# Hanbo-Cheng/DAWN-pytorch

Hardware: AMD Instinct MI355X
Metric: generated frames/sec at 256x256, 50 DDIM steps (higher is better)
Workload: dtype f32

## Files before the change

dawn-pytorch_amd/csrc/cond_xattn.hip:

```cpp
#include "dawn_common.h"
#include "../../include/dawn_hip.h"

namespace {

constexpr int XH = 8, XD = 8;
constexpr float XSCALE = 8.0f;

__global__ void xattn_prep_kernel(const float* __restrict__ kv, int F, const float* __restrict__ k_scale,
                                  const float* __restrict__ null_kv, float* __restrict__ kvtab, int branch,
                                  float* __restrict__ nulltab) {
    const int t = blockIdx.x * blockDim.x + threadIdx.x;
    if (t < F * XH) {
        const int f = t / XH, h = t % XH;
        const float* k = kv + (long)f * 128 + h * XD;
        const float* v = kv + (long)f * 128 + 64 + h * XD;
        float n2 = 0.f;
#pragma unroll
        for (int d = 0; d < XD; ++d) n2 += k[d] * k[d];
        const float inv = 1.0f / fmaxf(sqrtf(n2), 1e-12f);
        float* o = kvtab + ((long)f * 3 + branch) * 128;
#pragma unroll
        for (int d = 0; d < XD; ++d) {
            o[h * XD + d] = k[d] * inv * k_scale[d];
            o[64 + h * XD + d] = v[d];
// ... 57 lines not shown
__global__ __launch_bounds__(256) void xattn_ln_sum_kernel(const float* __restrict__ y3, const float* __restrict__ g3,
                                                           float* __restrict__ out, long rows, int Co, float eps) {
    constexpr int RPB = 256 / L;
    constexpr int MAXQ = 2;
    const int sub = threadIdx.x % L;
    const long row = (long)blockIdx.x * RPB + threadIdx.x / L;
    const bool ok = row < rows;
    const int nq = Co >> 2;
    f32x4 acc[MAXQ];
#pragma unroll
    for (int i = 0; i < MAXQ; ++i) acc[i] = f32x4{0.f, 0.f, 0.f, 0.f};
    for (int b = 0; b < 3; ++b) {
        const float* y = y3 + (row * 3 + b) * Co;
        f32x4 v[MAXQ];
        float s = 0.f;
#pragma unroll
        for (int i = 0; i < MAXQ; ++i) {
            const int qd = sub + i * L;
            v[i] = f32x4{0.f, 0.f, 0.f, 0.f};
            if (ok && qd < nq) {
                v[i] = *reinterpret_cast<const f32x4*>(y + qd * 4);
                s += v[i].x + v[i].y + v[i].z + v[i].w;
            }
        }
        s = wave_sum(s, L);
        const float mu = s / (float)Co;
        float ss = 0.f;
#pragma unroll
        for (int i = 0; i < MAXQ; ++i) {
            const int qd = sub + i * L;
            if (ok && qd < nq) {
                const f32x4 dl = v[i] - mu;
                ss += dl.x * dl.x + dl.y * dl.y + dl.z * dl.z + dl.w * dl.w;
            }
        }
        ss = wave_sum(ss, L);
        const float rs = rsqrtf(ss / (float)Co + eps);
#pragma unroll
        for (int i = 0; i < MAXQ; ++i) {
            const int qd = sub + i * L;
            if (ok && qd < nq) {
                const f32x4 g = *reinterpret_cast<const f32x4*>(g3 + b * Co + qd * 4);
                acc[i] += (v[i] - mu) * rs * g;
            }
        }
    }
#pragma unroll
    for (int i = 0; i < MAXQ; ++i) {
        const int qd = sub + i * L;
        if (ok && qd < nq) *reinterpret_cast<f32x4*>(out + row * Co + qd * 4) = acc[i];
    }
}

template <int L, int MAXQ>
__global__ __launch_bounds__(256) void xattn_sigma_out_kernel(const float* __restrict__ q, long rows, int HW,
                                                              const float* __restrict__ xtab, const float* __restrict__ g3,
                                                              int Co, float eps, float* out,
                                                              const float* gn_x , const float* __restrict__ gn_a,
                                                              const float* __restrict__ gn_b) {
    constexpr int RPB = 256 / L, R = 4;
    const int sub = threadIdx.x % L;
    const int lane = threadIdx.x & 63;
    const int gbase = lane - sub;
    const long row0 = ((long)blockIdx.x * RPB + threadIdx.x / L) * R;
    if (row0 >= rows) return;
    const int nq = Co >> 2;
    const int W = 64 + 9 * Co;
    const float* xt = xtab + (row0 / HW) * 3 * W;
    const int hd = sub & 7;
    f32x4 acc[R][MAXQ];
#pragma unroll
    for (int r = 0; r < R; ++r)
#pragma unroll
        for (int i = 0; i < MAXQ; ++i) acc[r][i] = f32x4{0.f, 0.f, 0.f, 0.f};
    const float rCo = 1.0f / (float)Co;
#pragma unroll 1
    for (int b = 0; b < 3; ++b) {
        const float* tb = xt + b * W;
        const f32x4 d0 = *reinterpret_cast<const f32x4*>(tb + hd * 8), d1 = *reinterpret_cast<const f32x4*>(tb + hd * 8 + 4);
        f32x4 u[9][MAXQ], g[MAXQ];
#pragma unroll
        for (int i = 0; i < MAXQ; ++i) {
            const int qd = sub + i * L;
            const bool ok = qd < nq;
#pragma unroll
            for (int k = 0; k < 9; ++k)
                u[k][i] = ok ? *reinterpret_cast<const f32x4*>(tb + 64 + k * Co + qd * 4) : f32x4{0.f, 0.f, 0.f, 0.f};
            g[i] = ok ? *reinterpret_cast<const f32x4*>(g3 + b * Co + qd * 4) : f32x4{0.f, 0.f, 0.f, 0.f};
        }
#pragma unroll
        for (int r = 0; r < R; ++r) {
            const float* qr = q + (row0 + r) * 192 + b * 64 + hd * 8;
            const f32x4 q0 = *reinterpret_cast<const f32x4*>(qr), q1 = *reinterpret_cast<const f32x4*>(qr + 4);
            const float n2 = (q0.x * q0.x + q0.y * q0.y + q0.z * q0.z + q0.w * q0.w) + (q1.x * q1.x + q1.y * q1.y + q1.z * q1.z + q1.w * q1.w);
            const float dd = (q0.x * d0.x + q0.y * d0.y + q0.z * d0.z + q0.w * d0.w) + (q1.x * d1.x + q1.y * d1.y + q1.z * d1.z + q1.w * d1.w);
            const float sg = __builtin_amdgcn_rcpf(1.0f + __builtin_amdgcn_exp2f(dd * __builtin_amdgcn_rsqf(fmaxf(n2, 1e-24f))));
            f32x4 y[MAXQ];
#pragma unroll
            for (int i = 0; i < MAXQ; ++i) y[i] = u[8][i];
#pragma unroll
            for (int k = 0; k < 8; ++k) {
                const float sk = __shfl(sg, gbase + k, 64);
#pragma unroll
                for (int i = 0; i < MAXQ; ++i) y[i] += u[k][i] * sk;
            }
            float s1 = 0.f;
#pragma unroll
            for (int i = 0; i < MAXQ; ++i) s1 += (y[i].x + y[i].y) + (y[i].z + y[i].w);
            const float mu = wave_sum(s1, L) * rCo;
            float s2 = 0.f;
#pragma unroll
            for (int i = 0; i < MAXQ; ++i) {
                if (sub + i * L < nq) {
                    const f32x4 dl = y[i] - mu;
                    s2 += (dl.x * dl.x + dl.y * dl.y) + (dl.z * dl.z + dl.w * dl.w);
                }
            }
            const float rs = __builtin_amdgcn_rsqf(wave_sum(s2, L) * rCo + eps);
#pragma unroll
            for (int i = 0; i < MAXQ; ++i) acc[r][i] += (y[i] - mu) * rs * g[i];
        }
    }
#pragma unroll
    for (int r = 0; r < R; ++r)
#pragma unroll
        for (int i = 0; i < MAXQ; ++i) {
            const int qd = sub + i * L;
            if (qd < nq) {
                f32x4 v = acc[r][i];
                if (gn_x) {
                    const f32x4 c4 = *reinterpret_cast<const f32x4*>(gn_x + (row0 + r) * Co + qd * 4);
                    const f32x4 a4 = *reinterpret_cast<const f32x4*>(gn_a + qd * 4), b4 = *reinterpret_cast<const f32x4*>(gn_b + qd * 4);
#pragma unroll
                    for (int j = 0; j < 4; ++j) v[j] = dawn_silu(c4[j] * a4[j] + b4[j]) + v[j];
                }
                *reinterpret_cast<f32x4*>(out + (row0 + r) * Co + qd * 4) = v;
            }
        }
}

}

extern "C" int dawn_xattn_sigma_out_h1(const float* q, long rows, int HW, const float* xtab, const float* g3, int Co, float eps,
                                       const float* gn_x, const float* gn_a, const float* gn_b, float* out, void* stream) {
    if (gn_x && (!gn_a || !gn_b)) return dawn_set_error_msg(-54, "dawn_xattn_sigma_out_h1: gn_x needs gn_a and gn_b");
    if (Co % 32 != 0 || Co < 32 || Co > 512 || HW % 4 != 0 || rows % 4 != 0)
        return dawn_set_error_msg(-53, "dawn_xattn_sigma_out: need Co % 32 == 0, 32 <= Co <= 512, H*W % 4 == 0");
    if (rows <= 0) return 0;
    hipStream_t s = (hipStream_t)stream;
    const int nq = Co / 4;
#define LAUNCH_XS(L, MQ)                                                                                                   \
    hipLaunchKernelGGL((xattn_sigma_out_kernel<L, MQ>), dim3(dawn_cdiv(rows, (256 / L) * 4)), dim3(256), 0, s, q, rows, HW, xtab, \
                       g3, Co, eps, out, gn_x, gn_a, gn_b)
    if (nq > 64) LAUNCH_XS(64, 2);
    else if (nq > 32) LAUNCH_XS(64, 1);
    else if (nq > 16) LAUNCH_XS(32, 1);
    else if (nq > 8) LAUNCH_XS(16, 1);
    else LAUNCH_XS(8, 1);
#undef LAUNCH_XS
    DAWN_LAUNCH_CHECK();
    return 0;
}
extern "C" int dawn_xattn_sigma_out(const float* q, long rows, int HW, const float* xtab, const float* g3, int Co, float eps,
                                    float* out, void* stream) {
    return dawn_xattn_sigma_out_h1(q, rows, HW, xtab, g3, Co, eps, nullptr, nullptr, nullptr, out, stream);
}

extern "C" int dawn_xattn_prep(const float* kv, int F, const float* k_scale, const float* null_kv, float* kvtab,
                               int branch, float* nulltab, void* stream) {
    hipLaunchKernelGGL(xattn_prep_kernel, dim3(dawn_cdiv((long)F * XH, 256)), dim3(256), 0, (hipStream_t)stream, kv, F,
                       k_scale, null_kv, kvtab, branch, nulltab);
    DAWN_LAUNCH_CHECK();
    return 0;
}
extern "C" int dawn_xattn_core(const float* q, float* o, long rows, int HW, const float* kvtab, const float* nulltab,
                               const float* q_scale, void* stream) {
    long total = rows * 24;
    int grid = (int)((total + 255) / 256);
    if (grid > 16384) grid = 16384;
    hipLaunchKernelGGL(xattn_core_kernel, dim3(grid), dim3(256), 0, (hipStream_t)stream, q, o, rows, HW, kvtab,
                       nulltab, q_scale);
    DAWN_LAUNCH_CHECK();
    return 0;
}
extern "C" int dawn_xattn_ln_sum(const float* y3, const float* g3, float* out, long rows, int Co, float eps,
                                 void* stream) {
    if (Co > 512 || Co % 4 != 0 || Co < 16) return dawn_set_error_msg(-50, "dawn_xattn_ln_sum: need 16 <= Co <= 512");
    hipStream_t s = (hipStream_t)stream;
    const int nq = Co / 4;
#define LAUNCH_XL(L)                                                                                            \
    hipLaunchKernelGGL(xattn_ln_sum_kernel<L>, dim3(dawn_cdiv(rows, 256 / L)), dim3(256), 0, s, y3, g3, out, rows, \
                       Co, eps)
    if (nq >= 64) LAUNCH_XL(64);
    else if (nq >= 32) LAUNCH_XL(32);
    else if (nq >= 16) LAUNCH_XL(16);
    else if (nq >= 8) LAUNCH_XL(8);
    else LAUNCH_XL(4);
#undef LAUNCH_XL
    DAWN_LAUNCH_CHECK();
    return 0;
}
```

dawn-pytorch_amd/csrc/sla_layer.hip:

```cpp
#include "dawn_common.h"
#include "../../include/dawn_hip.h"

namespace {

constexpr int C = 64;
constexpr int HEADS = 8;
constexpr int DH = 32;
constexpr int XLD = 68;
constexpr int QKVN = 3 * HEADS * DH;

__device__ __forceinline__ void stage_tile(const float* __restrict__ xf, int n0, int HW, float eps, float* Xt, int tid) {
    const int px = tid >> 4, sub = tid & 15;
    const int n = n0 + px;
    f32x4 v = {0.f, 0.f, 0.f, 0.f};
    if (n < HW) v = *reinterpret_cast<const f32x4*>(xf + (long)n * C + sub * 4);
    float s = v.x + v.y + v.z + v.w;
    s = wave_sum(s, 16);
    const float mu = s * (1.0f / C);
    const f32x4 dl = v - mu;
    float ss = dl.x * dl.x + dl.y * dl.y + dl.z * dl.z + dl.w * dl.w;
    ss = wave_sum(ss, 16);
    const float rs = 1.0f / sqrtf(ss * (1.0f / C) + eps);
    f32x4 o = dl * rs;
    if (n >= HW) o = f32x4{0.f, 0.f, 0.f, 0.f};
// ... 52 lines not shown
    stage_tile(xf, 0, HW, eps, Xs[0], tid);
    __syncthreads();
    for (int t = 0; t < ntiles; ++t) {
        if (t + 1 < ntiles) stage_tile(xf, 32 * (t + 1), HW, eps, Xs[(t + 1) & 1], tid);
        f32x16 kt = proj_N(Xs[t & 1], l31, half, wk);
        const f32x16 vt = proj_N(Xs[t & 1], l31, half, wv);
#pragma unroll
        for (int r = 0; r < 16; ++r) {
            const int n = 32 * t + (r & 3) + 8 * (r >> 2) + 4 * half;
            const float e = n < HW ? expf(kt[r] - mx) : 0.f;
            kt[r] = e;
            den += e;
        }
#pragma unroll
        for (int r = 0; r < 16; ++r) ctx = __builtin_amdgcn_mfma_f32_32x32x2f32(kt[r], vt[r], ctx, 0, 0, 0);
        __syncthreads();
    }
    den += __shfl_xor(den, 32, 64);
    float* dens = Xs[0];
    if (half == 0) dens[h * 32 + l31] = 1.0f / den;
    __syncthreads();
    float* ct = cT[h];
#pragma unroll
    for (int r = 0; r < 16; ++r) {
        const int d = (r & 3) + 8 * (r >> 2) + 4 * half;
        ct[d * 36 + l31] = ctx[r] * dens[h * 32 + d];
    }
    __syncthreads();
#pragma unroll
    for (int nt = 0; nt < 2; ++nt) {
        f32x16 m = zero16();
#pragma unroll
        for (int c = 0; c < 4; ++c) {
            const f32x4 a4 = *reinterpret_cast<const f32x4*>(ct + l31 * 36 + 8 * c + 4 * half);
            const f32x4 b4 = *reinterpret_cast<const f32x4*>(wout + ((size_t)(h * 8 + 2 * c + half) * C + 32 * nt + l31) * 4);
#pragma unroll
            for (int s = 0; s < 4; ++s) m = __builtin_amdgcn_mfma_f32_32x32x2f32(a4[s], b4[s], m, 0, 0, 0);
        }
        float* mo = Mout + (long)f * (HEADS * 8 * C * 4);
#pragma unroll
        for (int g = 0; g < 4; ++g)
            *reinterpret_cast<f32x4*>(mo + ((size_t)(h * 8 + 2 * g + half) * C + 32 * nt + l31) * 4) =
                f32x4{m[4 * g], m[4 * g + 1], m[4 * g + 2], m[4 * g + 3]};
    }
}


__device__ __forceinline__ f32x4 stage_load(const float* __restrict__ xf, int n0, int HW, int tid) {
    const int n = n0 + (tid >> 4);
    f32x4 v = {0.f, 0.f, 0.f, 0.f};
    if (n < HW) v = *reinterpret_cast<const f32x4*>(xf + (long)n * C + (tid & 15) * 4);
    return v;
}
__device__ __forceinline__ void stage_store(const f32x4 v, int n0, int HW, float eps, unsigned char* Pt, int tid) {
    const int px = tid >> 4, sub = tid & 15;
    const int n = n0 + px;
    float s = v.x + v.y + v.z + v.w;
    s = wave_sum(s, 16);
    const float mu = s * (1.0f / C);
    const f32x4 dl = v - mu;
    float ss = dl.x * dl.x + dl.y * dl.y + dl.z * dl.z + dl.w * dl.w;
    ss = wave_sum(ss, 16);
    const float rs = 1.0f / sqrtf(ss * (1.0f / C) + eps);
    f32x4 o = dl * rs;
    if (n >= HW) o = f32x4{0.f, 0.f, 0.f, 0.f};
    uint2 p1, p2, p3;
    dawn_split3_rne_quad(o, p1, p2, p3);
    const int kc = sub >> 2, qd = sub & 3;
    unsigned char* dst = Pt + ((size_t)((kc * 2 + (qd >> 1)) * 32 + px)) * 16 + (qd & 1) * 8;
    *reinterpret_cast<uint2*>(dst) = p1;
    *reinterpret_cast<uint2*>(dst + 4096) = p2;
    *reinterpret_cast<uint2*>(dst + 8192) = p3;
}

__global__ __launch_bounds__(512) void sla_c64_apply_kernel(const float* x , int HW,
                                                            const float* __restrict__ wqkv,
                                                            const float* __restrict__ Mg, const float* __restrict__ bias,
                                                            float eps, float* out, int nsplit) {
    extern __shared__ __attribute__((aligned(16))) float smem[];
    float* Wq = smem;
    float* Ms = smem + 16 * 256 * 4;
    const int tid = threadIdx.x;
    const int wave = tid >> 6, lane = tid & 63;
    const int l31 = lane & 31, half = lane >> 5;
    const int f = blockIdx.x / nsplit, sp = blockIdx.x % nsplit;
    for (int i = tid; i < 16 * 256; i += 512) {
        const int kq = i >> 8, n = i & 255;
        *reinterpret_cast<f32x4*>(Wq + i * 4) = *reinterpret_cast<const f32x4*>(wqkv + ((size_t)kq * QKVN + n) * 4);
    }
    const float* mf = Mg + (long)f * (HEADS * 8 * C * 4);
    for (int i = tid; i < 64 * 64; i += 512)
        *reinterpret_cast<f32x4*>(Ms + i * 4) = *reinterpret_cast<const f32x4*>(mf + (size_t)i * 4);
    __syncthreads();

    const int ntiles = (HW + 31) >> 5;
    const int per = (ntiles + nsplit - 1) / nsplit;
    const int t0 = sp * per, t1 = min(ntiles, t0 + per);
    const float scale = 0.17677669529663687f;
    for (int t = t0 + wave; t < t1; t += 8) {
        const int n = 32 * t + l31;
        const int nc = n < HW ? n : HW - 1;
        const float* xr = x + ((long)f * HW + nc) * C + 4 * half;
        f32x4 xb[8];
        float s = 0.f;
#pragma unroll
        for (int c = 0; c < 8; ++c) {
            xb[c] = *reinterpret_cast<const f32x4*>(xr + 8 * c);
            s += xb[c].x + xb[c].y + xb[c].z + xb[c].w;
        }
        s += __shfl_xor(s, 32, 64);
        const float mu = s * (1.0f / C);
        float ss = 0.f;
#pragma unroll
        for (int c = 0; c < 8; ++c) {
            const f32x4 dl = xb[c] - mu;
            ss += dl.x * dl.x + dl.y * dl.y + dl.z * dl.z + dl.w * dl.w;
        }
        ss += __shfl_xor(ss, 32, 64);
        const float rs = 1.0f / sqrtf(ss * (1.0f / C) + eps);
        f32x4 xn[8];
#pragma unroll
        for (int c = 0; c < 8; ++c) xn[c] = (xb[c] - mu) * rs;

        f32x16 oT[2];
        oT[0] = zero16();
// ... 178 lines not shown
                }
                l += __shfl_xor(l, 32, 64);
                const float inv = scale * __builtin_amdgcn_rcpf(l);
                if constexpr (OUTB) {
#pragma unroll
                    for (int j = 0; j < 2; ++j) {
                        float q8[8];
#pragma unroll
                        for (int i = 0; i < 8; ++i) q8[i] = qT[8 * j + i] * inv;
                        bf16x8 qb[3];
                        dawn_split3_oct(q8, qb[0], qb[1], qb[2]);
#pragma unroll
                        for (int nt = 0; nt < 2; ++nt) {
                            bf16x8 ma[3];
#pragma unroll
                            for (int pl = 0; pl < 3; ++pl)
                                ma[pl] = *reinterpret_cast<const bf16x8*>(Mp + ((size_t)((((h * 2 + j) * 3 + pl) * 2 + half) * C + 32 * nt + l31)) * 16);
#pragma unroll
                            for (int u = 0; u < 6; ++u)
                                oT[nt] = __builtin_amdgcn_mfma_f32_32x32x16_bf16(ma[DAWN_SPLIT6_A[u]], qb[DAWN_SPLIT6_B[u]], oT[nt], 0, 0, 0);
                        }
                    }
                } else {
#pragma unroll
                    for (int nt = 0; nt < 2; ++nt)
#pragma unroll
                        for (int c = 0; c < 4; ++c) {
                            const f32x4 a4 = *reinterpret_cast<const f32x4*>(Ms + ((h * 8 + 2 * c + half) * C + 32 * nt + l31) * 4);
#pragma unroll
                            for (int s2 = 0; s2 < 4; ++s2)
                                oT[nt] = __builtin_amdgcn_mfma_f32_32x32x2f32(a4[s2], qT[4 * c + s2] * inv, oT[nt], 0, 0, 0);
                        }
                }
            }
            if (n < HW) {
                const float* xrow = x + ((long)f * HW + n) * C;
                float* orow = out + ((long)f * HW + n) * C;
#pragma unroll
                for (int nt = 0; nt < 2; ++nt)
#pragma unroll
                    for (int g2 = 0; g2 < 4; ++g2) {
                        const int ch = 32 * nt + 8 * g2 + 4 * half;
                        const f32x4 b4 = *reinterpret_cast<const f32x4*>(bias + ch);
                        const f32x4 xres = *reinterpret_cast<const f32x4*>(xrow + ch);
                        f32x4 o = {oT[nt][4 * g2], oT[nt][4 * g2 + 1], oT[nt][4 * g2 + 2], oT[nt][4 * g2 + 3]};
                        *reinterpret_cast<f32x4*>(orow + ch) = o + b4 + xres;
                    }
            }
        }
        g += tB - tA;
    }
}

constexpr int SLA_PART = HEADS * (DH * DH + 2 * DH);

__device__ __forceinline__ void sla_ctx_proj(const unsigned char* Pt, int l31, int half, const bf16x8 (&wk)[4][3],
                                             const bf16x8 (&wv)[4][3], f32x16& kt, f32x16& vt) {
    kt = zero16();
    vt = zero16();
#pragma unroll
    for (int kc = 0; kc < 4; ++kc) {
        bf16x8 xa[3];
#pragma unroll
        for (int pl = 0; pl < 3; ++pl)
            xa[pl] = *reinterpret_cast<const bf16x8*>(Pt + pl * 4096 + ((size_t)((kc * 2 + half) * 32 + l31)) * 16);
#pragma unroll
        for (int u = 0; u < 6; ++u) {
            kt = __builtin_amdgcn_mfma_f32_32x32x16_bf16(xa[DAWN_SPLIT6_A[u]], wk[kc][DAWN_SPLIT6_B[u]], kt, 0, 0, 0);
            vt = __builtin_amdgcn_mfma_f32_32x32x16_bf16(xa[DAWN_SPLIT6_A[u]], wv[kc][DAWN_SPLIT6_B[u]], vt, 0, 0, 0);
        }
    }
}

template <bool FULL>
__device__ __forceinline__ void sla_ctx_post(f32x16& kt, const f32x16& vt, int t, int HW, int half, f32x16& ctx, float& den,
                                             float& mx) {
    constexpr float LOG2E = 1.4426950408889634f;
    float tm = -3.0e38f;
#pragma unroll
    for (int r = 0; r < 16; ++r) {
        const int n = 32 * t + (r & 3) + 8 * (r >> 2) + 4 * half;
        if (FULL || n < HW) tm = fmaxf(tm, kt[r]);
    }
    tm = fmaxf(tm, __shfl_xor(tm, 32, 64)) * LOG2E;
    if (__builtin_amdgcn_ballot_w64(tm > mx + 8.0f) != 0ull) {
        const float mnew = fmaxf(mx, tm);
        const float alpha = __builtin_amdgcn_exp2f(mx - mnew);
        den *= alpha;
#pragma unroll
        for (int r = 0; r < 16; ++r) {
            const int d0 = (r & 3) + 8 * (r >> 2);
            const float a0 = __builtin_bit_cast(float, __builtin_amdgcn_readlane(__builtin_bit_cast(int, alpha), d0));
            const float a1 = __builtin_bit_cast(float, __builtin_amdgcn_readlane(__builtin_bit_cast(int, alpha), d0 + 4));
            ctx[r] *= half ? a1 : a0;
        }
        mx = mnew;
    }
#pragma unroll
    for (int r = 0; r < 16; ++r) {
        const int n = 32 * t + (r & 3) + 8 * (r >> 2) + 4 * half;
        float e = __builtin_amdgcn_exp2f(__builtin_fmaf(kt[r], LOG2E, -mx));
        if (!FULL) e = n < HW ? e : 0.f;
        kt[r] = e;
        den += e;
    }
#pragma unroll
    for (int j = 0; j < 2; ++j) {
        float ek[8], vv[8];
#pragma unroll
        for (int i = 0; i < 8; ++i) { ek[i] = kt[8 * j + i]; vv[i] = vt[8 * j + i]; }
        bf16x8 e3[3], v3[3];
        dawn_split3_oct(ek, e3[0], e3[1], e3[2]);
        dawn_split3_oct(vv, v3[0], v3[1], v3[2]);
#pragma unroll
        for (int u = 0; u < 6; ++u) ctx = __builtin_amdgcn_mfma_f32_32x32x16_bf16(e3[DAWN_SPLIT6_A[u]], v3[DAWN_SPLIT6_B[u]], ctx, 0, 0, 0);
    }
}

__global__ __launch_bounds__(512) void sla_c64_context_part_kernel(const float* __restrict__ x, int HW,
                                                                   const unsigned short* __restrict__ wqkv_s, float eps,
                                                                   float* __restrict__ part, int ns, int per) {
    __shared__ __attribute__((aligned(16))) unsigned char Ps[2][12288];
    const int tid = threadIdx.x;
    const int h = tid >> 6, lane = tid & 63;
    const int l31 = lane & 31, half = lane >> 5;
    const int f = blockIdx.x / ns, sl = blockIdx.x - f * ns;
    const float* xf = x + (long)f * HW * C;
    const int ntiles = (HW + 31) >> 5;
    const int tA = sl * per, tB = min(ntiles, tA + per);

    bf16x8 wk[4][3], wv[4][3];
#pragma unroll
    for (int kc = 0; kc < 4; ++kc)
#pragma unroll
        for (int pl = 0; pl < 3; ++pl) {
            const size_t base = ((size_t)((kc * 3 + pl) * 2 + half) * QKVN) * 8;
            wk[kc][pl] = *reinterpret_cast<const bf16x8*>(wqkv_s + base + (size_t)(HEADS * DH + h * DH + l31) * 8);
            wv[kc][pl] = *reinterpret_cast<const bf16x8*>(wqkv_s + base + (size_t)(2 * HEADS * DH + h * DH + l31) * 8);
        }

    f32x16 ctx = zero16();
    float den = 0.f, mx = -3.0e38f;
    f32x4 vnext = {0.f, 0.f, 0.f, 0.f};
    if (tA < tB) stage_store(stage_load(xf, 32 * tA, HW, tid), 32 * tA, HW, eps, Ps[0], tid);
    if (tA + 1 < tB) vnext = stage_load(xf, 32 * (tA + 1), HW, tid);
    __syncthreads();
    f32x16 kt, vt;
    auto post = [&](int t) {
        if (32 * t + 32 <= HW) sla_ctx_post<true>(kt, vt, t, HW, half, ctx, den, mx);
        else sla_ctx_post<false>(kt, vt, t, HW, half, ctx, den, mx);
    };
    if (h < 4) {
        for (int t = tA; t < tB; ++t) {
            const f32x4 vcur = vnext;
            if (t + 2 < tB) vnext = stage_load(xf, 32 * (t + 2), HW, tid);
            sla_ctx_proj(Ps[(t - tA) & 1], l31, half, wk, wv, kt, vt);
            post(t);
            if (t + 1 < tB) stage_store(vcur, 32 * (t + 1), HW, eps, Ps[(t + 1 - tA) & 1], tid);
            __syncthreads();
        }
    } else {
        for (int t = tA; t < tB; ++t) {
            const f32x4 vcur = vnext;
            if (t + 2 < tB) vnext = stage_load(xf, 32 * (t + 2), HW, tid);
            if (t > tA) post(t - 1);
            if (t + 1 < tB) stage_store(vcur, 32 * (t + 1), HW, eps, Ps[(t + 1 - tA) & 1], tid);
            sla_ctx_proj(Ps[(t - tA) & 1], l31, half, wk, wv, kt, vt);
            __syncthreads();
        }
        if (tA < tB) post(tB - 1);
    }
    den += __shfl_xor(den, 32, 64);
    float* P = part + ((long)f * ns + sl) * SLA_PART;
#pragma unroll
    for (int r = 0; r < 16; ++r) {
        const int d = (r & 3) + 8 * (r >> 2) + 4 * half;
        P[h * (DH * DH) + d * DH + l31] = ctx[r];
    }
    if (half == 0) {
        P[HEADS * DH * DH + h * DH + l31] = den;
        P[HEADS * DH * DH + HEADS * DH + h * DH + l31] = mx;
    }
}

__global__ __launch_bounds__(512) void sla_c64_context_merge_kernel(const float* __restrict__ part, int ns,
                                                                    const float* __restrict__ wout, float* __restrict__ Mout) {
    __shared__ __attribute__((aligned(16))) float cT[HEADS][32 * 36];
    const int tid = threadIdx.x;
    const int h = tid >> 6, lane = tid & 63;
    const int l31 = lane & 31, half = lane >> 5;
    const int f = blockIdx.x;
    const float* P0 = part + (long)f * ns * SLA_PART;
    float* ct = cT[h];
    constexpr int OD = HEADS * DH * DH, OM = OD + HEADS * DH;
    float m[16], den[16], acc[16];
#pragma unroll
    for (int i = 0; i < 16; ++i) { m[i] = -3.0e38f; den[i] = 0.f; acc[i] = 0.f; }
    for (int sl = 0; sl < ns; ++sl) {
        const float* P = P0 + (long)sl * SLA_PART;
#pragma unroll
        for (int i = 0; i < 16; ++i) m[i] = fmaxf(m[i], P[OM + h * DH + 2 * i + half]);
    }
    for (int sl = 0; sl < ns; ++sl) {
        const float* P = P0 + (long)sl * SLA_PART;
#pragma unroll
        for (int i = 0; i < 16; ++i) {
            const int d = 2 * i + half;
            const float a = __builtin_amdgcn_exp2f(P[OM + h * DH + d] - m[i]);
            den[i] += a * P[OD + h * DH + d];
            acc[i] += a * P[h * (DH * DH) + d * DH + l31];
        }
    }
#pragma unroll
    for (int i = 0; i < 16; ++i) ct[(2 * i + half) * 36 + l31] = acc[i] * (1.0f / den[i]);
    __syncthreads();
#pragma unroll
    for (int nt = 0; nt < 2; ++nt) {
        f32x16 m = zero16();
#pragma unroll
        for (int c = 0; c < 4; ++c) {
            const f32x4 a4 = *reinterpret_cast<const f32x4*>(ct + l31 * 36 + 8 * c + 4 * half);
            const f32x4 b4 = *reinterpret_cast<const f32x4*>(wout + ((size_t)(h * 8 + 2 * c + half) * C + 32 * nt + l31) * 4);
#pragma unroll
            for (int s = 0; s < 4; ++s) m = __builtin_amdgcn_mfma_f32_32x32x2f32(a4[s], b4[s], m, 0, 0, 0);
        }
        float* mo = Mout + (long)f * (HEADS * 8 * C * 4);
#pragma unroll
        for (int g = 0; g < 4; ++g)
            *reinterpret_cast<f32x4*>(mo + ((size_t)(h * 8 + 2 * g + half) * C + 32 * nt + l31) * 4) =
                f32x4{m[4 * g], m[4 * g + 1], m[4 * g + 2], m[4 * g + 3]};
    }
}

int sla_ncu() {
    static int ncu = 0;
    if (!ncu) {
        int dev = 0, n = 0;
        if (hipGetDevice(&dev) != hipSuccess || hipDeviceGetAttribute(&n, hipDeviceAttributeMultiprocessorCount, dev) != hipSuccess || n <= 0)
            n = 256;
        ncu = n;
    }
    return ncu;
}

int sla_slices(int F, int HW) {
    const int ntiles = (HW + 31) / 32, ncu = sla_ncu();
    int best = 1;
    double bc = 1e30;
    for (int ns = 1; ns <= 8 && (ns == 1 || ntiles / ns >= 8); ++ns) {
        const double c = (double)(((long)F * ns + ncu - 1) / ncu) / ns + 0.01 * ns;
        if (c < bc - 1e-9) { bc = c; best = ns; }
    }
    return best;
}

}

extern "C" long dawn_sla_ws_floats(int F, int HW, int split) {
    return (long)F * (HEADS * 8 * C * 4) + (split ? (long)F * sla_slices(F, HW) * SLA_PART : 0);
}

extern "C" int dawn_sla_layer_c64(const float* x, int F, int HW, const float* wqkv, const void* wqkv_bf3,
                                  const float* wout, const float* bias, float eps, float* M_ws, float* out,
                                  void* stream) {
    if (F <= 0 || HW <= 0) return 0;
    hipStream_t s = (hipStream_t)stream;
    if (wqkv_bf3) {
        const int ns = sla_slices(F, HW), nt = (HW + 31) / 32;
        float* part = M_ws + (size_t)F * (HEADS * 8 * C * 4);
        hipLaunchKernelGGL(sla_c64_context_part_kernel, dim3(F * ns), dim3(512), 0, s, x, HW, (const unsigned short*)wqkv_bf3, eps,
                           part, ns, (nt + ns - 1) / ns);
        hipLaunchKernelGGL(sla_c64_context_merge_kernel, dim3(F), dim3(512), 0, s, part, ns, wout, M_ws);
    } else
        hipLaunchKernelGGL(sla_c64_context_kernel, dim3(F), dim3(512), 0, s, x, HW, wqkv, wout, eps, M_ws);
    const int ntiles = (HW + 31) / 32;
    if (wqkv_bf3) {
        const int ncu = sla_ncu();
        const long total = (long)F * ntiles;
        const int per = (int)((total + ncu - 1) / ncu);
        const int nblk = (int)((total + per - 1) / per);
#ifdef DAWN_SLA_OUT_FP32
        constexpr bool OUTB = false;
#else
        constexpr bool OUTB = true;
#endif
        const int lds = 160 * 1024;
        (void)hipFuncSetAttribute((const void*)sla_c64_apply_bf16_kernel<OUTB>, hipFuncAttributeMaxDynamicSharedMemorySize, lds);
        hipLaunchKernelGGL(sla_c64_apply_bf16_kernel<OUTB>, dim3(nblk), dim3(512), lds, s, x, HW, F, (const unsigned short*)wqkv_bf3,
                           M_ws, bias, eps, out, per);
    } else {
        const int nsplit = (ntiles >= 64) ? 2 : 1;
        const int lds = (16 * 256 * 4 + 64 * 64 * 4) * 4;
        (void)hipFuncSetAttribute((const void*)sla_c64_apply_kernel, hipFuncAttributeMaxDynamicSharedMemorySize, lds);
        hipLaunchKernelGGL(sla_c64_apply_kernel, dim3(F * nsplit), dim3(512), lds, s, x, HW, wqkv, M_ws, bias, eps, out,
                           nsplit);
    }
    DAWN_LAUNCH_CHECK();
    return 0;
}
```

Measured before the change: 173.2.

## Stage per-frame xattn tables in LDS and loop blocks over row runs

Rewrites the sigma-out cross-attention kernel so each block owns a run of rows inside one frame. The frame's key/value table and gamma are staged into shared memory once, and q and residual inputs are loaded through buffer loads with a software prefetch of the next row batch. Sigmoid gates are computed for several rows at once and broadcast with readlane or shfl. Group reductions now use DPP/permlane swaps instead of the generic wave_sum, and launch bounds add occupancy hints. In exchange it adds LDS pressure and more registers, and uses gfx950-specific permlane builtins.

```diff
diff --git a/dawn-pytorch_amd/csrc/cond_xattn.hip b/dawn-pytorch_amd/csrc/cond_xattn.hip
--- a/dawn-pytorch_amd/csrc/cond_xattn.hip
+++ b/dawn-pytorch_amd/csrc/cond_xattn.hip
@@ -133,91 +133,210 @@
     }
 }
 
+constexpr int xs_threads(int) { return 256; }
+constexpr int xs_waves(int l, int maxq) { return maxq > 1 ? 2 : l >= 32 ? 5 : l >= 16 ? 4 : 3; }
+template <int L>
+__device__ __forceinline__ float xs_group_sum(float v) {
+    if constexpr (L > 32) {
+        const auto p = __builtin_amdgcn_permlane32_swap(__float_as_uint(v), __float_as_uint(v), false, false);
+        v = __uint_as_float(p[0]) + __uint_as_float(p[1]);
+    }
+    if constexpr (L > 16) {
+        const auto p = __builtin_amdgcn_permlane16_swap(__float_as_uint(v), __float_as_uint(v), false, false);
+        v = __uint_as_float(p[0]) + __uint_as_float(p[1]);
+    }
+    if constexpr (L > 8) v += __int_as_float(__builtin_amdgcn_update_dpp(0, __float_as_int(v), 0x128, 0xf, 0xf, false));
+    if constexpr (L > 4) {
+        int t = __builtin_amdgcn_update_dpp(0, __float_as_int(v), 0x124, 0xf, 0xa, false);
+        t = __builtin_amdgcn_update_dpp(t, __float_as_int(v), 0x12c, 0xf, 0x5, false);
+        v += __int_as_float(t);
+    }
+    v += __int_as_float(__builtin_amdgcn_update_dpp(0, __float_as_int(v), 0x4e, 0xf, 0xf, false));
+    v += __int_as_float(__builtin_amdgcn_update_dpp(0, __float_as_int(v), 0xb1, 0xf, 0xf, false));
+    return v;
+}
+
+__device__ __forceinline__ float xs_sumsq(const f32x4 d) {
+#pragma clang fp contract(off)
+    return (d.x * d.x + d.y * d.y) + (d.z * d.z + d.w * d.w);
+}
+
 template <int L, int MAXQ>
-__global__ __launch_bounds__(256) void xattn_sigma_out_kernel(const float* __restrict__ q, long rows, int HW,
-                                                              const float* __restrict__ xtab, const float* __restrict__ g3,
-                                                              int Co, float eps, float* out,
-                                                              const float* gn_x , const float* __restrict__ gn_a,
-                                                              const float* __restrict__ gn_b) {
-    constexpr int RPB = 256 / L, R = 4;
+__global__ __launch_bounds__(xs_threads(MAXQ), xs_waves(L, MAXQ)) void xattn_sigma_out_kernel(const float* __restrict__ q, long rows, int HW, int run,
+                                                                   const float* __restrict__ xtab, const float* __restrict__ g3,
+                                                                   int Co, float eps, float* out,
+                                                                   const float* gn_x , const float* __restrict__ gn_a,
+                                                                   const float* __restrict__ gn_b) {
+    constexpr int NT = xs_threads(MAXQ), G = NT / L, R = 4;
+    constexpr int LG = L >= 32 ? 4 : L / 8;
+    constexpr int RS = R / LG;
+    __shared__ __attribute__((aligned(16))) float tab[3 * (64 + 10 * 4 * L * MAXQ)];
     const int sub = threadIdx.x % L;
     const int lane = threadIdx.x & 63;
     const int gbase = lane - sub;
-    const long row0 = ((long)blockIdx.x * RPB + threadIdx.x / L) * R;
-    if (row0 >= rows) return;
     const int nq = Co >> 2;
     const int W = 64 + 9 * Co;
-    const float* xt = xtab + (row0 / HW) * 3 * W;
-    const int hd = sub & 7;
-    f32x4 acc[R][MAXQ];
-#pragma unroll
-    for (int r = 0; r < R; ++r)
-#pragma unroll
-        for (int i = 0; i < MAXQ; ++i) acc[r][i] = f32x4{0.f, 0.f, 0.f, 0.f};
+    const int rpf = (HW + run - 1) / run;
+    const long f = blockIdx.x / rpf;
+    const int p0 = (int)(blockIdx.x - f * rpf) * run;
+    const long first = f * HW + p0;
+    const unsigned nrun = (unsigned)max(0L, min((long)(min(HW, p0 + run) - p0), rows - first));
+    const auto rq = DAWN_BUFFER(q + first * 192, nrun * 768u);
+    const auto rc = DAWN_BUFFER(gn_x ? gn_x + first * Co : nullptr, gn_x ? nrun * (unsigned)Co * 4u : 0u);
+    float* orun = out + first * Co;
+    unsigned row0 = (threadIdx.x / L) * R;
+    const int hd = sub & 7, sr = (sub >> 3) & (LG - 1);
+
+    f32x4 qa[RS][3][2], c4[R][MAXQ];
+    auto load_q = [&](unsigned r0) {
+#pragma unroll
+        for (int t = 0; t < RS; ++t)
+#pragma unroll
+            for (int b = 0; b < 3; ++b) {
+                const unsigned vo = (r0 + sr) * 768u + hd * 32;
+                qa[t][b][0] = __builtin_bit_cast(f32x4, __builtin_amdgcn_raw_buffer_load_b128(rq, vo, t * LG * 768 + b * 256, 0));
+                qa[t][b][1] = __builtin_bit_cast(f32x4, __builtin_amdgcn_raw_buffer_load_b128(rq, vo, t * LG * 768 + b * 256 + 16, 0));
+            }
+    };
+    auto load_c1 = [&](unsigned r0) {
+#pragma unroll
+        for (int r = 0; r < R; ++r)
+#pragma unroll
+            for (int i = 0; i < MAXQ; ++i) {
+                const int qd = sub + i * L;
+                const unsigned vo = qd < nq ? (r0 * (unsigned)Co + qd * 4) * 4u : 0x7fffffffu;
+                c4[r][i] = __builtin_bit_cast(f32x4, __builtin_amdgcn_raw_buffer_load_b128(rc, vo, r * Co * 4, 0));
+            }
+    };
+    bool act = row0 < nrun;
+    load_q(row0);
+    load_c1(row0);
+    {
+        const f32x4* src = reinterpret_cast<const f32x4*>(xtab + f * 3 * W);
+        const f32x4* gs = reinterpret_cast<const f32x4*>(g3);
+        f32x4* dst = reinterpret_cast<f32x4*>(tab);
+        const int n4 = (3 * W) >> 2;
+        for (int i = threadIdx.x; i < n4; i += NT) dst[i] = src[i];
+        for (int i = threadIdx.x; i < 3 * nq; i += NT) dst[n4 + i] = gs[i];
+    }
+    __syncthreads();
+    const float* gl = tab + 3 * W;
     const float rCo = 1.0f / (float)Co;
+    while (act) {
+        asm volatile("" ::: "memory");
+        float sg[RS][3];
+#pragma unroll
+        for (int t = 0; t < RS; ++t)
+#pragma unroll
+            for (int b = 0; b < 3; ++b) {
+                const f32x4 d0 = *reinterpret_cast<const f32x4*>(tab + b * W + hd * 8), d1 = *reinterpret_cast<const f32x4*>(tab + b * W + hd * 8 + 4);
+                const f32x4 q0 = qa[t][b][0], q1 = qa[t][b][1];
+                const float n2 = (q0.x * q0.x + q0.y * q0.y + q0.z * q0.z + q0.w * q0.w) + (q1.x * q1.x + q1.y * q1.y + q1.z * q1.z + q1.w * q1.w);
+                const float dd = (q0.x * d0.x + q0.y * d0.y + q0.z * d0.z + q0.w * d0.w) + (q1.x * d1.x + q1.y * d1.y + q1.z * d1.z + q1.w * d1.w);
+                sg[t][b] = __builtin_amdgcn_rcpf(1.0f + __builtin_amdgcn_exp2f(dd * __builtin_amdgcn_rsqf(fmaxf(n2, 1e-24f))));
+            }
+        const unsigned rown = row0 + G * R;
+        const bool actn = rown < nrun;
+        f32x4 acc[R][MAXQ];
+#pragma unroll
+        for (int r = 0; r < R; ++r)
+#pragma unroll
+            for (int i = 0; i < MAXQ; ++i) acc[r][i] = f32x4{0.f, 0.f, 0.f, 0.f};
 #pragma unroll 1
-    for (int b = 0; b < 3; ++b) {
-        const float* tb = xt + b * W;
-        const f32x4 d0 = *reinterpret_cast<const f32x4*>(tb + hd * 8), d1 = *reinterpret_cast<const f32x4*>(tb + hd * 8 + 4);
-        f32x4 u[9][MAXQ], g[MAXQ];
+        for (int b = 0; b < 3; ++b) {
+            const float* tb = tab + b * W + 64;
+            float sgb[RS];
+#pragma unroll
+            for (int t = 0; t < RS; ++t) sgb[t] = b == 0 ? sg[t][0] : b == 1 ? sg[t][1] : sg[t][2];
+            f32x4 y[R][MAXQ];
+#pragma unroll
+            for (int i = 0; i < MAXQ; ++i) {
+                const int qd = sub + i * L;
+                const f32x4 u8 = *reinterpret_cast<const f32x4*>(tb + 8 * Co + qd * 4);
+#pragma unroll
+                for (int r = 0; r < R; ++r) y[r][i] = u8;
+            }
+#pragma unroll
+            for (int k = 0; k < 8; ++k) {
+                f32x4 u[MAXQ];
+#pragma unroll
+                for (int i = 0; i < MAXQ; ++i) {
+                    const int qd = sub + i * L;
+                    u[i] = *reinterpret_cast<const f32x4*>(tb + k * Co + qd * 4);
+                }
+#pragma unroll
+                for (int r = 0; r < R; ++r) {
+                    float sk;
+                    if constexpr (L == 64) {
+                        sk = __int_as_float(__builtin_amdgcn_readlane(__float_as_int(sgb[0]), r * 8 + k));
+                    } else if constexpr (L == 32) {
+                        const float lo = __int_as_float(__builtin_amdgcn_readlane(__float_as_int(sgb[0]), r * 8 + k));
+                        const float hi = __int_as_float(__builtin_amdgcn_readlane(__float_as_int(sgb[0]), 32 + r * 8 + k));
+                        sk = gbase ? hi : lo;
+                    } else {
+                        sk = __shfl(sgb[r / LG], gbase + (r % LG) * 8 + k, 64);
+                    }
+#pragma unroll
+                    for (int i = 0; i < MAXQ; ++i) y[r][i] += u[i] * sk;
+                }
+            }
+            f32x4 g[MAXQ];
+#pragma unroll
+            for (int i = 0; i < MAXQ; ++i) {
+                const int qd = sub + i * L;
+                g[i] = *reinterpret_cast<const f32x4*>(gl + b * Co + qd * 4);
+            }
+#pragma unroll
+            for (int r = 0; r < R; ++r) {
+                float s1 = 0.f;
+#pragma unroll
+                for (int i = 0; i < MAXQ; ++i) s1 += sub + i * L < nq ? (y[r][i].x + y[r][i].y) + (y[r][i].z + y[r][i].w) : 0.f;
+                const float mu = xs_group_sum<L>(s1) * rCo;
+                float s2 = 0.f;
+#pragma unroll
+                for (int i = 0; i < MAXQ; ++i) {
+                    if (sub + i * L < nq) {
+                        const f32x4 dl = y[r][i] - mu;
+                        if constexpr (MAXQ == 1) s2 += xs_sumsq(dl);
+                        else s2 += (dl.x * dl.x + dl.y * dl.y) + (dl.z * dl.z + dl.w * dl.w);
+                    }
+                }
+                const float rs = __builtin_amdgcn_rsqf(xs_group_sum<L>(s2) * rCo + eps);
+#pragma unroll
+                for (int i = 0; i < MAXQ; ++i) acc[r][i] += (y[r][i] - mu) * rs * g[i];
+            }
+        }
+        f32x4 a4[MAXQ], b4[MAXQ];
 #pragma unroll
         for (int i = 0; i < MAXQ; ++i) {
             const int qd = sub + i * L;
-            const bool ok = qd < nq;
-#pragma unroll
-            for (int k = 0; k < 9; ++k)
-                u[k][i] = ok ? *reinterpret_cast<const f32x4*>(tb + 64 + k * Co + qd * 4) : f32x4{0.f, 0.f, 0.f, 0.f};
-            g[i] = ok ? *reinterpret_cast<const f32x4*>(g3 + b * Co + qd * 4) : f32x4{0.f, 0.f, 0.f, 0.f};
-        }
-#pragma unroll
-        for (int r = 0; r < R; ++r) {
-            const float* qr = q + (row0 + r) * 192 + b * 64 + hd * 8;
-            const f32x4 q0 = *reinterpret_cast<const f32x4*>(qr), q1 = *reinterpret_cast<const f32x4*>(qr + 4);
-            const float n2 = (q0.x * q0.x + q0.y * q0.y + q0.z * q0.z + q0.w * q0.w) + (q1.x * q1.x + q1.y * q1.y + q1.z * q1.z + q1.w * q1.w);
-            const float dd = (q0.x * d0.x + q0.y * d0.y + q0.z * d0.z + q0.w * d0.w) + (q1.x * d1.x + q1.y * d1.y + q1.z * d1.z + q1.w * d1.w);
-            const float sg = __builtin_amdgcn_rcpf(1.0f + __builtin_amdgcn_exp2f(dd * __builtin_amdgcn_rsqf(fmaxf(n2, 1e-24f))));
-            f32x4 y[MAXQ];
-#pragma unroll
-            for (int i = 0; i < MAXQ; ++i) y[i] = u[8][i];
-#pragma unroll
-            for (int k = 0; k < 8; ++k) {
-                const float sk = __shfl(sg, gbase + k, 64);
-#pragma unroll
-                for (int i = 0; i < MAXQ; ++i) y[i] += u[k][i] * sk;
-            }
-            float s1 = 0.f;
-#pragma unroll
-            for (int i = 0; i < MAXQ; ++i) s1 += (y[i].x + y[i].y) + (y[i].z + y[i].w);
-            const float mu = wave_sum(s1, L) * rCo;
-            float s2 = 0.f;
+            if (gn_x && qd < nq) a4[i] = *reinterpret_cast<const f32x4*>(gn_a + qd * 4), b4[i] = *reinterpret_cast<const f32x4*>(gn_b + qd * 4);
+        }
+#pragma unroll
+        for (int r = 0; r < R; ++r)
 #pragma unroll
             for (int i = 0; i < MAXQ; ++i) {
-                if (sub + i * L < nq) {
-                    const f32x4 dl = y[i] - mu;
-                    s2 += (dl.x * dl.x + dl.y * dl.y) + (dl.z * dl.z + dl.w * dl.w);
+                const int qd = sub + i * L;
+                if (qd < nq) {
+                    f32x4 v = acc[r][i];
+                    if (gn_x) {
+#pragma unroll
+                        for (int j = 0; j < 4; ++j) v[j] = dawn_silu(c4[r][i][j] * a4[i][j] + b4[i][j]) + v[j];
+                    }
+                    *reinterpret_cast<f32x4*>(orun + ((row0 + r) * (unsigned)Co + qd * 4)) = v;
                 }
             }
-            const float rs = __builtin_amdgcn_rsqf(wave_sum(s2, L) * rCo + eps);
-#pragma unroll
-            for (int i = 0; i < MAXQ; ++i) acc[r][i] += (y[i] - mu) * rs * g[i];
-        }
-    }
-#pragma unroll
-    for (int r = 0; r < R; ++r)
-#pragma unroll
-        for (int i = 0; i < MAXQ; ++i) {
-            const int qd = sub + i * L;
-            if (qd < nq) {
-                f32x4 v = acc[r][i];
-                if (gn_x) {
-                    const f32x4 c4 = *reinterpret_cast<const f32x4*>(gn_x + (row0 + r) * Co + qd * 4);
-                    const f32x4 a4 = *reinterpret_cast<const f32x4*>(gn_a + qd * 4), b4 = *reinterpret_cast<const f32x4*>(gn_b + qd * 4);
-#pragma unroll
-                    for (int j = 0; j < 4; ++j) v[j] = dawn_silu(c4[j] * a4[j] + b4[j]) + v[j];
-                }
-                *reinterpret_cast<f32x4*>(out + (row0 + r) * Co + qd * 4) = v;
-            }
-        }
+        load_q(rown);
+        load_c1(rown);
+        row0 = rown;
+        act = actn;
+    }
+}
+
+int xattn_run_rows(int step_rows, long frames, int HW) {
+    int run = step_rows > 128 ? step_rows : 128;
+    while (run > step_rows && frames * dawn_cdiv(HW, run) < 1024) run >>= 1;
+    return run;
 }
 
 }
@@ -230,9 +349,13 @@
     if (rows <= 0) return 0;
     hipStream_t s = (hipStream_t)stream;
     const int nq = Co / 4;
+    const long frames = (rows + HW - 1) / HW;
 #define LAUNCH_XS(L, MQ)                                                                                                   \
-    hipLaunchKernelGGL((xattn_sigma_out_kernel<L, MQ>), dim3(dawn_cdiv(rows, (256 / L) * 4)), dim3(256), 0, s, q, rows, HW, xtab, \
-                       g3, Co, eps, out, gn_x, gn_a, gn_b)
+    do {                                                                                                                   \
+        const int run = xattn_run_rows((xs_threads(MQ) / L) * 4, frames, HW);                                              \
+        hipLaunchKernelGGL((xattn_sigma_out_kernel<L, MQ>), dim3((unsigned)(frames * dawn_cdiv(HW, run))), dim3(xs_threads(MQ)), 0, s, \
+                           q, rows, HW, run, xtab, g3, Co, eps, out, gn_x, gn_a, gn_b);                                    \
+    } while (0)
     if (nq > 64) LAUNCH_XS(64, 2);
     else if (nq > 32) LAUNCH_XS(64, 1);
     else if (nq > 16) LAUNCH_XS(32, 1);
@@ -246,6 +369,7 @@
                                     float* out, void* stream) {
     return dawn_xattn_sigma_out_h1(q, rows, HW, xtab, g3, Co, eps, nullptr, nullptr, nullptr, out, stream);
 }
+
 
 extern "C" int dawn_xattn_prep(const float* kv, int F, const float* k_scale, const float* null_kv, float* kvtab,
                                int branch, float* nulltab, void* stream) {
```

Measured after the change: 174.6 (median of 6 runs). Within noise of the previous version (+0.8%).

## Defer V projection in SLA context: accumulate softmax(K)·X, apply Wv in merge

Applied to the files above, without the earlier changes.

The context-partial kernel no longer projects V per tile. It accumulates exp(K)-weighted sums of the normalized input (a 32x64 Gram-like matrix per head) using a transposed LDS copy of the split-bf16 tile, and the merge kernel multiplies by Wv once per frame. This removes half of the per-tile projection MFMAs and the V split, trading them for larger partial buffers, an extra transposed staging write built with permlane swaps, and a small extra matmul in merge. It also XOR-swizzles LDS slots to reduce bank conflicts and switches the reductions to row16_sum.

```diff
diff --git a/dawn-pytorch_amd/csrc/sla_layer.hip b/dawn-pytorch_amd/csrc/sla_layer.hip
--- a/dawn-pytorch_amd/csrc/sla_layer.hip
+++ b/dawn-pytorch_amd/csrc/sla_layer.hip
@@ -128,25 +128,38 @@
     if (n < HW) v = *reinterpret_cast<const f32x4*>(xf + (long)n * C + (tid & 15) * 4);
     return v;
 }
-__device__ __forceinline__ void stage_store(const f32x4 v, int n0, int HW, float eps, unsigned char* Pt, int tid) {
+__device__ __forceinline__ int sla_tslot(int c) { return c ^ ((c >> 3) & 3); }
+__device__ __forceinline__ uint2 sla_px_transpose(const uint2 p) {
+    const auto s1 = __builtin_amdgcn_permlane32_swap(p.x, p.y, false, false);
+    const unsigned a = s1[0], b = s1[1];
+    const auto s2 = __builtin_amdgcn_permlane16_swap(__builtin_amdgcn_perm(b, a, 0x05040100u), __builtin_amdgcn_perm(b, a, 0x07060302u),
+                                                     false, false);
+    return uint2{__builtin_amdgcn_perm(s2[1], s2[0], 0x05040100u), __builtin_amdgcn_perm(s2[1], s2[0], 0x07060302u)};
+}
+__device__ __forceinline__ void stage_store(const f32x4 v, int n0, int HW, float eps, unsigned char* Pt, unsigned char* Tt, int tid) {
     const int px = tid >> 4, sub = tid & 15;
     const int n = n0 + px;
     float s = v.x + v.y + v.z + v.w;
-    s = wave_sum(s, 16);
+    s = row16_sum(s);
     const float mu = s * (1.0f / C);
     const f32x4 dl = v - mu;
     float ss = dl.x * dl.x + dl.y * dl.y + dl.z * dl.z + dl.w * dl.w;
-    ss = wave_sum(ss, 16);
+    ss = row16_sum(ss);
     const float rs = 1.0f / sqrtf(ss * (1.0f / C) + eps);
     f32x4 o = dl * rs;
     if (n >= HW) o = f32x4{0.f, 0.f, 0.f, 0.f};
     uint2 p1, p2, p3;
     dawn_split3_rne_quad(o, p1, p2, p3);
     const int kc = sub >> 2, qd = sub & 3;
-    unsigned char* dst = Pt + ((size_t)((kc * 2 + (qd >> 1)) * 32 + px)) * 16 + (qd & 1) * 8;
+    unsigned char* dst = Pt + ((size_t)((kc * 2 + (qd >> 1)) * 32 + (px ^ ((kc * 2 + (qd >> 1)) & 3)))) * 16 + (qd & 1) * 8;
     *reinterpret_cast<uint2*>(dst) = p1;
     *reinterpret_cast<uint2*>(dst + 4096) = p2;
     *reinterpret_cast<uint2*>(dst + 8192) = p3;
+    const int w = tid >> 6, q = (tid >> 4) & 3;
+    unsigned char* dt = Tt + ((size_t)(((w >> 2) * 2 + (w & 1)) * C + sla_tslot(4 * sub + q))) * 16 + ((w >> 1) & 1) * 8;
+    *reinterpret_cast<uint2*>(dt) = sla_px_transpose(p1);
+    *reinterpret_cast<uint2*>(dt + 4096) = sla_px_transpose(p2);
+    *reinterpret_cast<uint2*>(dt + 8192) = sla_px_transpose(p3);
 }
 
 __global__ __launch_bounds__(512) void sla_c64_apply_kernel(const float* x , int HW,
@@ -431,29 +444,25 @@
     }
 }
 
-constexpr int SLA_PART = HEADS * (DH * DH + 2 * DH);
-
-__device__ __forceinline__ void sla_ctx_proj(const unsigned char* Pt, int l31, int half, const bf16x8 (&wk)[4][3],
-                                             const bf16x8 (&wv)[4][3], f32x16& kt, f32x16& vt) {
+constexpr int SLA_PART = HEADS * (DH * C + 2 * DH);
+
+__device__ __forceinline__ void sla_ctx_proj(const unsigned char* Pt, int l31, int half, const bf16x8 (&wk)[4][3], f32x16& kt) {
     kt = zero16();
-    vt = zero16();
 #pragma unroll
     for (int kc = 0; kc < 4; ++kc) {
         bf16x8 xa[3];
 #pragma unroll
         for (int pl = 0; pl < 3; ++pl)
-            xa[pl] = *reinterpret_cast<const bf16x8*>(Pt + pl * 4096 + ((size_t)((kc * 2 + half) * 32 + l31)) * 16);
-#pragma unroll
-        for (int u = 0; u < 6; ++u) {
+            xa[pl] = *reinterpret_cast<const bf16x8*>(Pt + pl * 4096 + ((size_t)((kc * 2 + half) * 32 + (l31 ^ ((kc * 2 + half) & 3)))) * 16);
+#pragma unroll
+        for (int u = 0; u < 6; ++u)
             kt = __builtin_amdgcn_mfma_f32_32x32x16_bf16(xa[DAWN_SPLIT6_A[u]], wk[kc][DAWN_SPLIT6_B[u]], kt, 0, 0, 0);
-            vt = __builtin_amdgcn_mfma_f32_32x32x16_bf16(xa[DAWN_SPLIT6_A[u]], wv[kc][DAWN_SPLIT6_B[u]], vt, 0, 0, 0);
-        }
     }
 }
 
 template <bool FULL>
-__device__ __forceinline__ void sla_ctx_post(f32x16& kt, const f32x16& vt, int t, int HW, int half, f32x16& ctx, float& den,
-                                             float& mx) {
+__device__ __forceinline__ void sla_ctx_post(f32x16& kt, const unsigned char* Tt, int t, int HW, int l31, int half, f32x16 (&G)[2],
+                                             float& den, float& mx) {
     constexpr float LOG2E = 1.4426950408889634f;
     float tm = -3.0e38f;
 #pragma unroll
@@ -471,7 +480,8 @@
             const int d0 = (r & 3) + 8 * (r >> 2);
             const float a0 = __builtin_bit_cast(float, __builtin_amdgcn_readlane(__builtin_bit_cast(int, alpha), d0));
             const float a1 = __builtin_bit_cast(float, __builtin_amdgcn_readlane(__builtin_bit_cast(int, alpha), d0 + 4));
-            ctx[r] *= half ? a1 : a0;
+            G[0][r] *= half ? a1 : a0;
+            G[1][r] *= half ? a1 : a0;
         }
         mx = mnew;
     }
@@ -485,14 +495,21 @@
     }
 #pragma unroll
     for (int j = 0; j < 2; ++j) {
-        float ek[8], vv[8];
-#pragma unroll
-        for (int i = 0; i < 8; ++i) { ek[i] = kt[8 * j + i]; vv[i] = vt[8 * j + i]; }
-        bf16x8 e3[3], v3[3];
+        float ek[8];
+#pragma unroll
+        for (int i = 0; i < 8; ++i) ek[i] = kt[8 * j + i];
+        bf16x8 e3[3];
         dawn_split3_oct(ek, e3[0], e3[1], e3[2]);
-        dawn_split3_oct(vv, v3[0], v3[1], v3[2]);
-#pragma unroll
-        for (int u = 0; u < 6; ++u) ctx = __builtin_amdgcn_mfma_f32_32x32x16_bf16(e3[DAWN_SPLIT6_A[u]], v3[DAWN_SPLIT6_B[u]], ctx, 0, 0, 0);
+#pragma unroll
+        for (int nb = 0; nb < 2; ++nb) {
+            bf16x8 xb[3];
+#pragma unroll
+            for (int pl = 0; pl < 3; ++pl)
+                xb[pl] = *reinterpret_cast<const bf16x8*>(Tt + pl * 4096 + ((size_t)((j * 2 + half) * C + sla_tslot(32 * nb + l31))) * 16);
+#pragma unroll
+            for (int u = 0; u < 6; ++u)
+                G[nb] = __builtin_amdgcn_mfma_f32_32x32x16_bf16(e3[DAWN_SPLIT6_A[u]], xb[DAWN_SPLIT6_B[u]], G[nb], 0, 0, 0);
+        }
     }
 }
 
@@ -500,6 +517,7 @@
                                                                    const unsigned short* __restrict__ wqkv_s, float eps,
                                                                    float* __restrict__ part, int ns, int per) {
     __shared__ __attribute__((aligned(16))) unsigned char Ps[2][12288];
+    __shared__ __attribute__((aligned(16))) unsigned char Ts[3][12288];
     const int tid = threadIdx.x;
     const int h = tid >> 6, lane = tid & 63;
     const int l31 = lane & 31, half = lane >> 5;
@@ -508,34 +526,32 @@
     const int ntiles = (HW + 31) >> 5;
     const int tA = sl * per, tB = min(ntiles, tA + per);
 
-    bf16x8 wk[4][3], wv[4][3];
+    bf16x8 wk[4][3];
 #pragma unroll
     for (int kc = 0; kc < 4; ++kc)
 #pragma unroll
-        for (int pl = 0; pl < 3; ++pl) {
-            const size_t base = ((size_t)((kc * 3 + pl) * 2 + half) * QKVN) * 8;
-            wk[kc][pl] = *reinterpret_cast<const bf16x8*>(wqkv_s + base + (size_t)(HEADS * DH + h * DH + l31) * 8);
-            wv[kc][pl] = *reinterpret_cast<const bf16x8*>(wqkv_s + base + (size_t)(2 * HEADS * DH + h * DH + l31) * 8);
-        }
-
-    f32x16 ctx = zero16();
+        for (int pl = 0; pl < 3; ++pl)
+            wk[kc][pl] = *reinterpret_cast<const bf16x8*>(wqkv_s + ((size_t)((kc * 3 + pl) * 2 + half) * QKVN + HEADS * DH + h * DH + l31) * 8);
+
+    f32x16 G[2] = {zero16(), zero16()};
     float den = 0.f, mx = -3.0e38f;
     f32x4 vnext = {0.f, 0.f, 0.f, 0.f};
-    if (tA < tB) stage_store(stage_load(xf, 32 * tA, HW, tid), 32 * tA, HW, eps, Ps[0], tid);
+    if (tA < tB) stage_store(stage_load(xf, 32 * tA, HW, tid), 32 * tA, HW, eps, Ps[0], Ts[0], tid);
     if (tA + 1 < tB) vnext = stage_load(xf, 32 * (tA + 1), HW, tid);
     __syncthreads();
-    f32x16 kt, vt;
+    f32x16 kt;
     auto post = [&](int t) {
-        if (32 * t + 32 <= HW) sla_ctx_post<true>(kt, vt, t, HW, half, ctx, den, mx);
-        else sla_ctx_post<false>(kt, vt, t, HW, half, ctx, den, mx);
+        const unsigned char* Tt = Ts[(t - tA) % 3];
+        if (32 * t + 32 <= HW) sla_ctx_post<true>(kt, Tt, t, HW, l31, half, G, den, mx);
+        else sla_ctx_post<false>(kt, Tt, t, HW, l31, half, G, den, mx);
     };
     if (h < 4) {
         for (int t = tA; t < tB; ++t) {
             const f32x4 vcur = vnext;
             if (t + 2 < tB) vnext = stage_load(xf, 32 * (t + 2), HW, tid);
-            sla_ctx_proj(Ps[(t - tA) & 1], l31, half, wk, wv, kt, vt);
+            sla_ctx_proj(Ps[(t - tA) & 1], l31, half, wk, kt);
             post(t);
-            if (t + 1 < tB) stage_store(vcur, 32 * (t + 1), HW, eps, Ps[(t + 1 - tA) & 1], tid);
+            if (t + 1 < tB) stage_store(vcur, 32 * (t + 1), HW, eps, Ps[(t + 1 - tA) & 1], Ts[(t + 1 - tA) % 3], tid);
             __syncthreads();
         }
     } else {
@@ -543,71 +559,84 @@
             const f32x4 vcur = vnext;
             if (t + 2 < tB) vnext = stage_load(xf, 32 * (t + 2), HW, tid);
             if (t > tA) post(t - 1);
-            if (t + 1 < tB) stage_store(vcur, 32 * (t + 1), HW, eps, Ps[(t + 1 - tA) & 1], tid);
-            sla_ctx_proj(Ps[(t - tA) & 1], l31, half, wk, wv, kt, vt);
+            if (t + 1 < tB) stage_store(vcur, 32 * (t + 1), HW, eps, Ps[(t + 1 - tA) & 1], Ts[(t + 1 - tA) % 3], tid);
+            sla_ctx_proj(Ps[(t - tA) & 1], l31, half, wk, kt);
             __syncthreads();
         }
         if (tA < tB) post(tB - 1);
     }
     den += __shfl_xor(den, 32, 64);
-    float* P = part + ((long)f * ns + sl) * SLA_PART;
-#pragma unroll
-    for (int r = 0; r < 16; ++r) {
-        const int d = (r & 3) + 8 * (r >> 2) + 4 * half;
-        P[h * (DH * DH) + d * DH + l31] = ctx[r];
+    float* P = part + ((long)f * ns + sl) * SLA_PART + h * (DH * C);
+#pragma unroll
+    for (int nb = 0; nb < 2; ++nb) {
+        const int c = 32 * nb + l31;
+#pragma unroll
+        for (int r = 0; r < 16; ++r) {
+            const int d = (r & 3) + 8 * (r >> 2) + 4 * half;
+            P[((c >> 2) * DH + d) * 4 + (c & 3)] = G[nb][r];
+        }
     }
     if (half == 0) {
-        P[HEADS * DH * DH + h * DH + l31] = den;
-        P[HEADS * DH * DH + HEADS * DH + h * DH + l31] = mx;
+        part[((long)f * ns + sl) * SLA_PART + HEADS * DH * C + h * DH + l31] = den;
+        part[((long)f * ns + sl) * SLA_PART + HEADS * DH * C + HEADS * DH + h * DH + l31] = mx;
     }
 }
 
 __global__ __launch_bounds__(512) void sla_c64_context_merge_kernel(const float* __restrict__ part, int ns,
+                                                                    const float* __restrict__ wqkv,
                                                                     const float* __restrict__ wout, float* __restrict__ Mout) {
     __shared__ __attribute__((aligned(16))) float cT[HEADS][32 * 36];
+    __shared__ float dens[HEADS][DH];
     const int tid = threadIdx.x;
     const int h = tid >> 6, lane = tid & 63;
     const int l31 = lane & 31, half = lane >> 5;
     const int f = blockIdx.x;
     const float* P0 = part + (long)f * ns * SLA_PART;
     float* ct = cT[h];
-    constexpr int OD = HEADS * DH * DH, OM = OD + HEADS * DH;
-    float m[16], den[16], acc[16];
-#pragma unroll
-    for (int i = 0; i < 16; ++i) { m[i] = -3.0e38f; den[i] = 0.f; acc[i] = 0.f; }
+    constexpr int OD = HEADS * DH * C, OM = OD + HEADS * DH;
+    float m = -3.0e38f, den = 0.f;
+    for (int sl = 0; sl < ns; ++sl) m = fmaxf(m, P0[(long)sl * SLA_PART + OM + h * DH + l31]);
+    f32x4 g[8];
+#pragma unroll
+    for (int cc = 0; cc < 8; ++cc) g[cc] = f32x4{0.f, 0.f, 0.f, 0.f};
     for (int sl = 0; sl < ns; ++sl) {
         const float* P = P0 + (long)sl * SLA_PART;
-#pragma unroll
-        for (int i = 0; i < 16; ++i) m[i] = fmaxf(m[i], P[OM + h * DH + 2 * i + half]);
-    }
-    for (int sl = 0; sl < ns; ++sl) {
-        const float* P = P0 + (long)sl * SLA_PART;
-#pragma unroll
-        for (int i = 0; i < 16; ++i) {
-            const int d = 2 * i + half;
-            const float a = __builtin_amdgcn_exp2f(P[OM + h * DH + d] - m[i]);
-            den[i] += a * P[OD + h * DH + d];
-            acc[i] += a * P[h * (DH * DH) + d * DH + l31];
-        }
-    }
-#pragma unroll
-    for (int i = 0; i < 16; ++i) ct[(2 * i + half) * 36 + l31] = acc[i] * (1.0f / den[i]);
+        const float a = __builtin_amdgcn_exp2f(P[OM + h * DH + l31] - m);
+        den += a * P[OD + h * DH + l31];
+#pragma unroll
+        for (int cc = 0; cc < 8; ++cc)
+            g[cc] += *reinterpret_cast<const f32x4*>(P + h * (DH * C) + ((2 * cc + half) * DH + l31) * 4) * a;
+    }
+    f32x16 ctx = zero16();
+#pragma unroll
+    for (int cc = 0; cc < 8; ++cc) {
+        const f32x4 b4 = *reinterpret_cast<const f32x4*>(wqkv + ((size_t)(2 * cc + half) * QKVN + 2 * HEADS * DH + h * DH + l31) * 4);
+#pragma unroll
+        for (int s = 0; s < 4; ++s) ctx = __builtin_amdgcn_mfma_f32_32x32x2f32(g[cc][s], b4[s], ctx, 0, 0, 0);
+    }
+    if (half == 0) dens[h][l31] = 1.0f / den;
     __syncthreads();
 #pragma unroll
+    for (int r = 0; r < 16; ++r) {
+        const int d = (r & 3) + 8 * (r >> 2) + 4 * half;
+        ct[d * 36 + l31] = ctx[r] * dens[h][d];
+    }
+    __syncthreads();
+#pragma unroll
     for (int nt = 0; nt < 2; ++nt) {
-        f32x16 m = zero16();
+        f32x16 mo16 = zero16();
 #pragma unroll
         for (int c = 0; c < 4; ++c) {
             const f32x4 a4 = *reinterpret_cast<const f32x4*>(ct + l31 * 36 + 8 * c + 4 * half);
             const f32x4 b4 = *reinterpret_cast<const f32x4*>(wout + ((size_t)(h * 8 + 2 * c + half) * C + 32 * nt + l31) * 4);
 #pragma unroll
-            for (int s = 0; s < 4; ++s) m = __builtin_amdgcn_mfma_f32_32x32x2f32(a4[s], b4[s], m, 0, 0, 0);
+            for (int s = 0; s < 4; ++s) mo16 = __builtin_amdgcn_mfma_f32_32x32x2f32(a4[s], b4[s], mo16, 0, 0, 0);
         }
         float* mo = Mout + (long)f * (HEADS * 8 * C * 4);
 #pragma unroll
-        for (int g = 0; g < 4; ++g)
-            *reinterpret_cast<f32x4*>(mo + ((size_t)(h * 8 + 2 * g + half) * C + 32 * nt + l31) * 4) =
-                f32x4{m[4 * g], m[4 * g + 1], m[4 * g + 2], m[4 * g + 3]};
+        for (int g2 = 0; g2 < 4; ++g2)
+            *reinterpret_cast<f32x4*>(mo + ((size_t)(h * 8 + 2 * g2 + half) * C + 32 * nt + l31) * 4) =
+                f32x4{mo16[4 * g2], mo16[4 * g2 + 1], mo16[4 * g2 + 2], mo16[4 * g2 + 3]};
     }
 }
 
@@ -649,7 +678,7 @@
         float* part = M_ws + (size_t)F * (HEADS * 8 * C * 4);
         hipLaunchKernelGGL(sla_c64_context_part_kernel, dim3(F * ns), dim3(512), 0, s, x, HW, (const unsigned short*)wqkv_bf3, eps,
                            part, ns, (nt + ns - 1) / ns);
-        hipLaunchKernelGGL(sla_c64_context_merge_kernel, dim3(F), dim3(512), 0, s, part, ns, wout, M_ws);
+        hipLaunchKernelGGL(sla_c64_context_merge_kernel, dim3(F), dim3(512), 0, s, part, ns, wqkv, wout, M_ws);
     } else
         hipLaunchKernelGGL(sla_c64_context_kernel, dim3(F), dim3(512), 0, s, x, HW, wqkv, wout, eps, M_ws);
     const int ntiles = (HW + 31) / 32;
```

Result: no change. 177.2 before, 176.7 after (-0.3%).
